# QZ1-boy/CDFO

Measured on NVIDIA B200. Metric: HR frames/sec, 1080p x4 LD-QP37, higher is better.
Workload: dtype bf16

## Files before the change

cdfo_b200/config.py:

```python
import os

tensor_core = True

dcn_gather = "tex"

conv_pair = os.environ.get("CDFO_CONV_PAIR", "1") != "0"

conv_fold_half = os.environ.get("CDFO_CONV_FOLD_HALF", "1") != "0"

conv_parity_planes = os.environ.get("CDFO_CONV_PARITY_PLANES", "1") != "0"
trunk_fused_resample = os.environ.get("CDFO_TRUNK_FUSED_RESAMPLE", "1") != "0"

head_dual = os.environ.get("CDFO_HEAD_DUAL", "1") != "0"

fused_head_dcn = os.environ.get("CDFO_FUSED_HEAD_DCN", "1") != "0"

features_c8 = os.environ.get("CDFO_FEATURES_C8", "1") != "0"
mdta_c8 = os.environ.get("CDFO_MDTA_C8", "1") != "0"
trunk_compose_1x1 = os.environ.get("CDFO_TRUNK_COMPOSE_1X1", "1") != "0"
trunk_fused_upsample = os.environ.get("CDFO_TRUNK_FUSED_UPSAMPLE", "1") != "0"
lra_logits_from_prior = os.environ.get("CDFO_LRA_LOGITS_FROM_PRIOR", "1") != "0"
```

cdfo_b200/csrc/lra.cu:

```cuda
#include <cuda.h>
#include <cstring>

#include "cdfo_common.cuh"
#include "sm100_ptx.cuh"

namespace cdfo {

__device__ __forceinline__ float warp_max(float v) {
#pragma unroll
  for (int o = 16; o > 0; o >>= 1) v = fmaxf(v, __shfl_xor_sync(0xffffffffu, v, o));
  return v;
}
__device__ __forceinline__ float warp_sum(float v) {
#pragma unroll
  for (int o = 16; o > 0; o >>= 1) v += __shfl_xor_sync(0xffffffffu, v, o);
  return v;
}

__global__ void lra_mask_kernel(const float *__restrict__ u, const float *__restrict__ vmax, const float *__restrict__ qv,
                                uint8_t *__restrict__ midx, float *__restrict__ qsel, int HW) {
  __shared__ float vm[64];
  const int b = blockIdx.y;
  if (threadIdx.x < 64) vm[threadIdx.x] = vmax[b * 64 + threadIdx.x];
  __syncthreads();
// ... 641 lines not shown
    for (int r = 0; r < 2; ++r) {
      l_run[r] += __shfl_xor_sync(0xffffffffu, l_run[r], 1);
      l_run[r] += __shfl_xor_sync(0xffffffffu, l_run[r], 2);
    }
    const float inv0 = 1.f / l_run[0], inv1 = 1.f / l_run[1];
    const int h0 = q0 + g, h1 = q0 + g + 8;
#pragma unroll
    for (int n = 0; n < 8; ++n) {
      if (h0 < H) *reinterpret_cast<float2 *>(long_out + (((size_t)b * H + h0) * W + w) * 64 + 8 * n + 2 * tq) = make_float2(o[n][0] * inv0, o[n][1] * inv0);
      if (h1 < H) *reinterpret_cast<float2 *>(long_out + (((size_t)b * H + h1) * W + w) * 64 + 8 * n + 2 * tq) = make_float2(o[n][2] * inv1, o[n][3] * inv1);
    }
  }
}

constexpr int kWinThreads = 256;
__global__ void __launch_bounds__(kWinThreads) lra_win_kernel(const float *__restrict__ qv, const uint8_t *__restrict__ midx,
                                                             float *__restrict__ loc_out, int H, int W) {
  extern __shared__ __align__(16) float sm[];
  float *q = sm;
  float *v = q + 64 * kLd;
  float *Ps = v + 64 * kLd;
  const int b = blockIdx.z, wy = blockIdx.y, wx = blockIdx.x;
  const int HW = H * W;
  const int tid = threadIdx.x;
  static_assert(kWinThreads == 256, "one token and 16 + 16 channels per thread");
  {
    const int tok = tid & 63, cg = tid >> 6;
    const int h = wy * 8 + (tok >> 3), w = wx * 8 + (tok & 7);
    const size_t pix = (size_t)h * W + w;
    const int cm = midx[(size_t)b * HW + pix];
    const float *qp = qv + ((size_t)b * 128 + cg) * HW + pix;
    float qr[16], vv[16];
#pragma unroll
    for (int k = 0; k < 16; ++k) {
      qr[k] = __ldg(qp + (size_t)(4 * k) * HW);
      vv[k] = __ldg(qp + (size_t)(64 + 4 * k) * HW);
    }
#pragma unroll
    for (int k = 0; k < 16; ++k) {
      const int c = 4 * k + cg;
      q[tok * kLd + c] = cm == c ? 0.f : qr[k];
      v[tok * kLd + c] = vv[k];
    }
  }
  __syncthreads();
  const float *Kcur = q;
  flash_block_fp32_kptr(q, &Kcur, v, Ps, 64, [&](int) {}, [&](int tok, int c4, float4 val) {
    const int h = wy * 8 + (tok >> 3), w = wx * 8 + (tok & 7);
    *reinterpret_cast<float4 *>(loc_out + (((size_t)b * H + h) * W + w) * 64 + c4) = val;
  });
}

constexpr int kWinTcThreads = 128, kWinLd = 36;
__global__ void __launch_bounds__(kWinTcThreads, 6) lra_win_tc_kernel(const float *__restrict__ qv, const uint8_t *__restrict__ midx,
                                                                      float *__restrict__ loc_out, int H, int W) {
  __shared__ uint32_t Qh[64 * kWinLd], Ql[64 * kWinLd], Vt[64 * kWinLd], Vl[64 * kWinLd];
  const int b = blockIdx.z, wy = blockIdx.y, wx = blockIdx.x;
  const int HW = H * W;
  const int tid = threadIdx.x, lane = tid & 31, warp = tid >> 5, g = lane >> 2, tq = lane & 3;
  {
    const int tok = tid & 63, half = tid >> 6;
    const int h = wy * 8 + (tok >> 3), w = wx * 8 + (tok & 7);
    const size_t pix = (size_t)h * W + w;
    const int cm = midx[(size_t)b * HW + pix];
    const float *qp = qv + ((size_t)b * 128 + half * 32) * HW + pix;
#pragma unroll 4
    for (int k = 0; k < 16; ++k) {
      const int c = half * 32 + 2 * k;
      float q0 = __ldg(qp + (size_t)(2 * k) * HW), q1 = __ldg(qp + (size_t)(2 * k + 1) * HW);
      if (cm == c) q0 = 0.f;
      if (cm == c + 1) q1 = 0.f;
      const __nv_bfloat16 h0 = __float2bfloat16_rn(q0), h1 = __float2bfloat16_rn(q1);
      Qh[tok * kWinLd + (c >> 1)] = pack_bf16x2(__bfloat162float(h0), __bfloat162float(h1));
      Ql[tok * kWinLd + (c >> 1)] = pack_bf16x2(q0 - __bfloat162float(h0), q1 - __bfloat162float(h1));
      const float v0 = __ldg(qp + (size_t)(64 + 2 * k) * HW), v1 = __ldg(qp + (size_t)(64 + 2 * k + 1) * HW);
      const __nv_bfloat16 vh0 = __float2bfloat16_rn(v0), vh1 = __float2bfloat16_rn(v1);
      reinterpret_cast<__nv_bfloat16 *>(Vt)[(c * kWinLd) * 2 + tok] = vh0;
      reinterpret_cast<__nv_bfloat16 *>(Vt)[((c + 1) * kWinLd) * 2 + tok] = vh1;
      reinterpret_cast<__nv_bfloat16 *>(Vl)[(c * kWinLd) * 2 + tok] = __float2bfloat16_rn(v0 - __bfloat162float(vh0));
      reinterpret_cast<__nv_bfloat16 *>(Vl)[((c + 1) * kWinLd) * 2 + tok] = __float2bfloat16_rn(v1 - __bfloat162float(vh1));
    }
  }
  __syncthreads();
  const int q0r = warp * 16;
  uint32_t ah[4][4], al[4][4];
#pragma unroll
  for (int s = 0; s < 4; ++s) {
    ah[s][0] = Qh[(q0r + g) * kWinLd + 8 * s + tq];      ah[s][1] = Qh[(q0r + g + 8) * kWinLd + 8 * s + tq];
    ah[s][2] = Qh[(q0r + g) * kWinLd + 8 * s + tq + 4];  ah[s][3] = Qh[(q0r + g + 8) * kWinLd + 8 * s + tq + 4];
    al[s][0] = Ql[(q0r + g) * kWinLd + 8 * s + tq];      al[s][1] = Ql[(q0r + g + 8) * kWinLd + 8 * s + tq];
    al[s][2] = Ql[(q0r + g) * kWinLd + 8 * s + tq + 4];  al[s][3] = Ql[(q0r + g + 8) * kWinLd + 8 * s + tq + 4];
  }
  float sc[8][4];
#pragma unroll
  for (int n = 0; n < 8; ++n) {
#pragma unroll
    for (int i = 0; i < 4; ++i) sc[n][i] = 0.f;
    const uint32_t *kh_ = Qh + (8 * n + g) * kWinLd + tq, *kl_ = Ql + (8 * n + g) * kWinLd + tq;
#pragma unroll
    for (int s = 0; s < 4; ++s) {
      const uint32_t bh0 = kh_[8 * s], bh1 = kh_[8 * s + 4];
      mma_bf16(sc[n], al[s], bh0, bh1);
      mma_bf16(sc[n], ah[s], kl_[8 * s], kl_[8 * s + 4]);
      mma_bf16(sc[n], ah[s], bh0, bh1);
    }
  }
  float mx[2] = {-INFINITY, -INFINITY}, sum[2] = {0.f, 0.f};
#pragma unroll
  for (int n = 0; n < 8; ++n) {
    mx[0] = fmaxf(mx[0], fmaxf(sc[n][0], sc[n][1]));
    mx[1] = fmaxf(mx[1], fmaxf(sc[n][2], sc[n][3]));
  }
#pragma unroll
  for (int r = 0; r < 2; ++r) {
    mx[r] = fmaxf(mx[r], __shfl_xor_sync(0xffffffffu, mx[r], 1));
    mx[r] = fmaxf(mx[r], __shfl_xor_sync(0xffffffffu, mx[r], 2));
  }
#pragma unroll
  for (int n = 0; n < 8; ++n) {
    sc[n][0] = expf(sc[n][0] - mx[0]); sc[n][1] = expf(sc[n][1] - mx[0]);
    sc[n][2] = expf(sc[n][2] - mx[1]); sc[n][3] = expf(sc[n][3] - mx[1]);
    sum[0] += sc[n][0] + sc[n][1];
    sum[1] += sc[n][2] + sc[n][3];
  }
  float o[8][4];
#pragma unroll
  for (int n = 0; n < 8; ++n)
#pragma unroll
    for (int i = 0; i < 4; ++i) o[n][i] = 0.f;
#pragma unroll
  for (int s = 0; s < 4; ++s) {
    uint32_t ap[4], apl[4];
#pragma unroll
    for (int i = 0; i < 4; ++i) {
      const float p0 = sc[2 * s + (i >> 1)][2 * (i & 1)], p1 = sc[2 * s + (i >> 1)][2 * (i & 1) + 1];
      const float h0 = __bfloat162float(__float2bfloat16_rn(p0)), h1 = __bfloat162float(__float2bfloat16_rn(p1));
      ap[i] = pack_bf16x2(h0, h1);
      apl[i] = pack_bf16x2(p0 - h0, p1 - h1);
    }
    const uint32_t *vr = Vt + g * kWinLd + 8 * s + tq, *vl = Vl + g * kWinLd + 8 * s + tq;
#pragma unroll
    for (int n = 0; n < 8; ++n) {
      const uint32_t b0 = vr[8 * n * kWinLd], b1 = vr[8 * n * kWinLd + 4];
      mma_bf16(o[n], apl, b0, b1);
      mma_bf16(o[n], ap, vl[8 * n * kWinLd], vl[8 * n * kWinLd + 4]);
      mma_bf16(o[n], ap, b0, b1);
    }
  }
#pragma unroll
  for (int r = 0; r < 2; ++r) {
    sum[r] += __shfl_xor_sync(0xffffffffu, sum[r], 1);
    sum[r] += __shfl_xor_sync(0xffffffffu, sum[r], 2);
  }
  const float inv0 = 1.f / sum[0], inv1 = 1.f / sum[1];
  const int t0 = q0r + g, t1 = t0 + 8;
  float *d0 = loc_out + (((size_t)b * H + wy * 8 + (t0 >> 3)) * W + wx * 8 + (t0 & 7)) * 64 + 2 * tq;
  float *d1 = loc_out + (((size_t)b * H + wy * 8 + (t1 >> 3)) * W + wx * 8 + (t1 & 7)) * 64 + 2 * tq;
#pragma unroll
  for (int n = 0; n < 8; ++n) {
    *reinterpret_cast<float2 *>(d0 + 8 * n) = make_float2(o[n][0] * inv0, o[n][1] * inv0);
    *reinterpret_cast<float2 *>(d1 + 8 * n) = make_float2(o[n][2] * inv1, o[n][3] * inv1);
  }
}

}

using namespace cdfo;

typedef CUresult (*LraEncodeTiledFn)(CUtensorMap *, CUtensorMapDataType, cuuint32_t, void *, const cuuint64_t *, const cuuint64_t *,
                                     const cuuint32_t *, const cuuint32_t *, CUtensorMapInterleave, CUtensorMapSwizzle,
                                     CUtensorMapL2promotion, CUtensorMapFloatOOBfill);
static LraEncodeTiledFn lra_encode_tiled_fn() {
  static LraEncodeTiledFn fn = nullptr;
  if (!fn) {
    void *ptr = nullptr;
    cudaDriverEntryPointQueryResult q;
    if (cudaGetDriverEntryPoint("cuTensorMapEncodeTiled", &ptr, cudaEnableDefault, &q) == cudaSuccess && q == cudaDriverEntryPointSuccess)
      fn = reinterpret_cast<LraEncodeTiledFn>(ptr);
  }
  return fn;
}

static bool g_lra_row_tma = true;
extern "C" int cdfo_lra_set_row_tma(int on) {
  g_lra_row_tma = on != 0;
  return CDFO_OK;
}
static bool g_lra_col_tf32 = false;
static bool g_lra_col_tc = true;
static bool g_lra_win_tc = true;
extern "C" int cdfo_lra_set_col_precision(int tf32) {
  g_lra_col_tf32 = tf32 != 0;
  return CDFO_OK;
}
extern "C" int cdfo_lra_set_col_tcgen05(int on) {
  g_lra_col_tc = on != 0;
  return CDFO_OK;
}
extern "C" int cdfo_lra_set_win_tensor_core(int on) {
  g_lra_win_tc = on != 0;
  return CDFO_OK;
}

extern "C" size_t cdfo_lra_workspace_bytes(int B, int H, int W) {
  const size_t P = (size_t)B * H * W;
  return P * (1 + 4) + 3 * P * 64 * 4 + 256;
}

static int lra_run(const float *qv, const float *u, const float *vmax, const float *x, const float *x2, const float *tables,
                   float beta, float bh, const float *fuse_w, const float *fuse_b, float *out, void *out_c8, int out_channels,
                   int channel0, void *workspace, int B, int H, int W, void *stream);

extern "C" int cdfo_lra_fwd(const float *qv, const float *u, const float *vmax, const float *x, const float *x2, const float *tables,
                            float beta, float bh, const float *fuse_w, const float *fuse_b, float *out, void *workspace, int B,
                            int H, int W, void *stream) {
  return lra_run(qv, u, vmax, x, x2, tables, beta, bh, fuse_w, fuse_b, out, nullptr, 0, 0, workspace, B, H, W, stream);
}

extern "C" int cdfo_lra_c8_fwd(const float *qv, const float *u, const float *vmax, const float *x, const float *x2, const float *tables,
                               float beta, float bh, const float *fuse_w, const float *fuse_b, void *out_c8, int out_channels,
                               int channel0, void *workspace, int B, int H, int W, void *stream) {
  CDFO_REQUIRE(out_c8 && ((uintptr_t)out_c8 & 15) == 0, CDFO_ERR_NULL, "cdfo_lra_c8_fwd: out_c8 must be a 16-byte aligned pointer");
  CDFO_REQUIRE(out_channels % 8 == 0 && channel0 % 8 == 0 && channel0 >= 0 && channel0 + 64 <= out_channels, CDFO_ERR_SHAPE,
               "cdfo_lra_c8_fwd: channels [%d, %d) do not fit %d output channels (multiples of 8)", channel0, channel0 + 64, out_channels);
  return lra_run(qv, u, vmax, x, x2, tables, beta, bh, fuse_w, fuse_b, nullptr, out_c8, out_channels, channel0, workspace, B, H, W, stream);
}

static int lra_run(const float *qv, const float *u, const float *vmax, const float *x, const float *x2, const float *tables,
                   float beta, float bh, const float *fuse_w, const float *fuse_b, float *out, void *out_c8, int out_channels,
                   int channel0, void *workspace, int B, int H, int W, void *stream) {
  CDFO_REQUIRE(qv && u && vmax && x && tables && fuse_w && fuse_b && (out || out_c8) && workspace, CDFO_ERR_NULL, "cdfo_lra_fwd: NULL pointer");
  CDFO_REQUIRE(B > 0 && B <= 65535 && H > 0 && W > 0 && H % 8 == 0 && W % 8 == 0, CDFO_ERR_SHAPE,
               "cdfo_lra_fwd: H and W must be multiples of the window size 8 (got %d x %d)", H, W);
  cudaStream_t s = (cudaStream_t)stream;
  const size_t P = (size_t)B * H * W;
  const int HW = H * W;
  uint8_t *ws = (uint8_t *)workspace;
  float *qsel = (float *)ws;
  float *vrow_t = qsel + P;
  float *long_out = vrow_t + P * 64;
  float *loc_out = long_out + P * 64;
  uint8_t *midx = (uint8_t *)(loc_out + P * 64);
  LraTables t{tables, tables + 9, tables + 18, tables + 82, beta, bh};

  lra_mask_kernel<<<dim3(ceil_div(HW, 128), B), 128, 0, s>>>(u, vmax, qv, midx, qsel, HW);

  const int Wk = (W + 63) & ~63;
  const size_t row_smem = ((size_t)Wk * kLd + 4096 + 3 * (size_t)Wk + 64 + kRowThreads + 2 * (size_t)Wk) * 4;
  const int Hk = (H + 63) & ~63;
  const size_t col_v = (size_t)Hk * kLd > (size_t)(H + 8) * 64 ? (size_t)Hk * kLd : (size_t)(H + 8) * 64;
  const size_t col_smem = ((size_t)Hk * kLd + col_v) * 4;
  const size_t win_smem = (size_t)3 * 64 * kLd * 4;
  const int kDynMax = 224 * 1024;
  CDFO_REQUIRE(row_smem <= (size_t)kDynMax && col_smem <= (size_t)kDynMax, CDFO_ERR_UNSUPPORTED,
               "cdfo_lra_fwd: frame %d x %d exceeds the shared-memory row/column buffers (W <= 704, H <= 384)", H, W);
  static bool attr = false;
  if (!attr) {
    cudaError_t e1 = cudaFuncSetAttribute(lra_row_kernel<false>, cudaFuncAttributeMaxDynamicSharedMemorySize, kDynMax);
    if (e1 == cudaSuccess) e1 = cudaFuncSetAttribute(lra_row_kernel<true>, cudaFuncAttributeMaxDynamicSharedMemorySize, kDynMax);
    cudaError_t e2 = cudaFuncSetAttribute(lra_col_kernel, cudaFuncAttributeMaxDynamicSharedMemorySize, kDynMax);
    if (e2 == cudaSuccess) e2 = cudaFuncSetAttribute(lra_col_bf16_kernel, cudaFuncAttributeMaxDynamicSharedMemorySize, kDynMax);
    cudaError_t e3 = cudaFuncSetAttribute(lra_win_kernel, cudaFuncAttributeMaxDynamicSharedMemorySize, (int)win_smem);
    if (e1 != cudaSuccess || e2 != cudaSuccess || e3 != cudaSuccess)
      return fail(CDFO_ERR_CUDA, "cdfo_lra_fwd: cudaFuncSetAttribute failed: %s", cudaGetErrorString(e1 != cudaSuccess ? e1 : (e2 != cudaSuccess ? e2 : e3)));
    attr = true;
  }
  {
    CUtensorMap qm;
    memset(&qm, 0, sizeof(qm));
    bool row_tma = g_lra_row_tma && W % 4 == 0 && ((uintptr_t)qv & 15) == 0 && row_smem + kRowRawBytes <= (size_t)kDynMax;
    if (row_tma) {
      static LraEncodeTiledFn enc = lra_encode_tiled_fn();
      if (enc) {
        const cuuint64_t gdim[3] = {(cuuint64_t)W, (cuuint64_t)H, (cuuint64_t)B * 128};
        const cuuint64_t gstr[2] = {(cuuint64_t)W * 4, (cuuint64_t)H * W * 4};
        const cuuint32_t box[3] = {kRowPiece, 1, 64};
        const cuuint32_t estr[3] = {1, 1, 1};
        CUresult cr = enc(&qm, CU_TENSOR_MAP_DATA_TYPE_FLOAT32, 3, const_cast<float *>(qv), gdim, gstr, box, estr, CU_TENSOR_MAP_INTERLEAVE_NONE,
                          CU_TENSOR_MAP_SWIZZLE_NONE, CU_TENSOR_MAP_L2_PROMOTION_L2_128B, CU_TENSOR_MAP_FLOAT_OOB_FILL_NONE);
        CDFO_REQUIRE(cr == CUDA_SUCCESS, CDFO_ERR_CUDA, "cuTensorMapEncodeTiled(qv rows) failed with CUresult %d", (int)cr);
      } else {
        row_tma = false;
      }
    }
    if (row_tma) lra_row_kernel<true><<<dim3(H, B), kRowThreads, row_smem + kRowRawBytes, s>>>(qm, qv, midx, qsel, vrow_t, t, H, W);
    else lra_row_kernel<false><<<dim3(H, B), kRowThreads, row_smem, s>>>(qm, qv, midx, qsel, vrow_t, t, H, W);
  }
  int col_done = 0;
  if (!g_lra_col_tf32 && g_lra_col_tc) {
    col_done = lra_col_sm100_launch(vrow_t, midx, qsel, long_out, t, B, H, W, s);
    if (col_done < 0) return col_done;
  }
  if (col_done) {
  } else if (g_lra_col_tf32) {
    lra_col_kernel<<<dim3(W, B), kColThreads, col_smem, s>>>(vrow_t, midx, qsel, long_out, t, H, W);
  } else {
    const size_t col16_smem = ((size_t)Hk * kQw + 64 * ((size_t)Hk / 2 + 4) + 2 * (size_t)(H + 8) + 16) * 4;
    lra_col_bf16_kernel<<<dim3(W, B), kColThreads, col16_smem, s>>>(vrow_t, midx, qsel, long_out, t, H, W);
  }
  if (g_lra_win_tc) lra_win_tc_kernel<<<dim3(W / 8, H / 8, B), kWinTcThreads, 0, s>>>(qv, midx, loc_out, H, W);
  else lra_win_kernel<<<dim3(W / 8, H / 8, B), kWinThreads, win_smem, s>>>(qv, midx, loc_out, H, W);
  if (int rc = check_launch("cdfo_lra_fwd")) return rc;
  return pointwise_conv(long_out, loc_out, fuse_w, fuse_b, x, x2, out, B, 128, 64, HW, 0, 1, s, out_c8, out_channels, channel0);
}
```

cdfo_b200/hotpath.py:

```python
import ctypes

import torch
import torch.nn.functional as F

from . import _lib, config, conv, dcn_sm100


def _lrelu(x):
    return F.leaky_relu(x, 0.1)


def _c(mod, x, **kw):
    return F.conv2d(x, mod.weight, mod.bias, **kw)


def _pkey(*params):
    return tuple((p.data_ptr(), str(p.device), p._version, p.dtype) for p in params)


def _module_cache(mod, slot, key, build):
    store = mod.__dict__.setdefault("_cdfo_derived", {})
    hit = store.get(slot)
    if hit is not None and hit[0] == key:
        return hit[1]
# ... 157 lines not shown
        k1 = tapm.sum(dim=1)
        r = tapm @ tapm.t()
        tab = torch.cat([kw, kh, k1, r.reshape(-1)]).float().contiguous()
        return tab, float(mod.directW1_conv.bias.detach()), float(mod.directH1_conv.bias.detach())
    return _module_cache(mod, "lra_tables", _pkey(mod.directW1_conv.weight, mod.directH1_conv.weight, mod.directW1_conv.bias,
                                                   mod.directH1_conv.bias), build)


@torch.no_grad()
def mask_logits(mod, v):
    B, C, H, W = v.shape
    if C != 64:
        raise _lib.CdfoError("mask_logits: 64 channels expected")
    c2, c3 = mod.conv_du_re._modules["2"], mod.conv_du_re2._modules["0"]
    ws = torch.empty(_lib.lib().cdfo_lra_mask_logits_workspace_bytes(B, H, W), dtype=torch.uint8, device=v.device)
    vmax = torch.empty((B, 64), dtype=torch.float32, device=v.device)
    _lib.call("cdfo_lra_mask_logits_fwd", _lib.ptr(_f32(v)), _lib.ptr(_f32(c2.weight)), _lib.ptr(_f32(c2.bias)), _lib.ptr(_f32(c3.weight).reshape(64, 64)),
              _lib.ptr(_f32(c3.bias)), _lib.ptr(vmax), _lib.ptr(ws), B, H, W, _lib.stream_ptr(v.device))
    return vmax


def _pointwise(in1, in2, weight, bias, act, mode=0, resid1=None, resid2=None):
    B, K, H, W = in1.shape
    Co = weight.size(0)
    out = torch.empty((B, Co, H, W), dtype=torch.float32, device=in1.device)
    _lib.call("cdfo_pointwise_conv_fwd", _lib.ptr(in1), _lib.ptr(in2), _lib.ptr(_f32(weight).reshape(Co, -1)), _lib.ptr(None if bias is None else _f32(bias)),
              _lib.ptr(resid1), _lib.ptr(resid2), _lib.ptr(out), B, K, Co, H, W, int(act), int(mode), _lib.stream_ptr(in1.device))
    return out


@torch.no_grad()
def long_range_attention(mod, res, x, u, x2=None, out8=None, channel0=0, res_prior=None):
    B, C, H, W = x.shape
    x = _f32(x)
    x2 = None if x2 is None else _f32(x2)
    du0 = mod.conv_du_re._modules["0"]
    if res_prior is not None:
        pc, rms1 = res_prior

        def build():
            w1 = du0.weight.detach().float().reshape(64, 64)
            return (w1 @ pc.weight.detach().float().reshape(64, 9)).contiguous(), (w1 @ pc.bias.detach().float() + du0.bias.detach().float()).contiguous()
        wv, bv = _module_cache(mod, "du0_after_prior", _pkey(du0.weight, du0.bias, pc.weight, pc.bias), build)
        rms1 = _f32(rms1)
        v = torch.empty((B, 64, H, W), dtype=torch.float32, device=x.device)
        _lib.call("cdfo_prior_conv_act_fwd", _lib.ptr(rms1), _lib.ptr(wv), _lib.ptr(bv), _lib.ptr(v), B, 64, H, W, 1, _lib.stream_ptr(x.device))
    else:
        v = _pointwise(_f32(res), None, du0.weight, du0.bias, act=1)
    vmax = mask_logits(mod, v)
    qv = _pointwise(x, x2, mod.input_conv.weight, mod.input_conv.bias, act=0)
    nbytes = _lib.lib().cdfo_lra_workspace_bytes(B, H, W)
    ws = torch.empty(nbytes, dtype=torch.uint8, device=x.device)
    tab, beta, bh = _lra_tap_tables(mod)
    if out8 is not None:
        if out8.dtype != torch.bfloat16 or not out8.is_contiguous() or out8.dim() != 5 or (out8.size(0), out8.size(2), out8.size(3), out8.size(4)) != (B, H, W, 8):
            raise _lib.CdfoError("long_range_attention: out8 must be a contiguous bf16 c8 tensor of the same batch and size")
        _lib.call("cdfo_lra_c8_fwd", _lib.ptr(qv), _lib.ptr(u.contiguous()), _lib.ptr(vmax), _lib.ptr(x), _lib.ptr(x2), _lib.ptr(tab),
                  ctypes.c_float(beta), ctypes.c_float(bh),
                  _lib.ptr(_f32(mod.fuse.weight).reshape(64, 128)), _lib.ptr(_f32(mod.fuse.bias)),
                  _lib.ptr(out8), out8.size(1) * 8, int(channel0), _lib.ptr(ws), B, H, W, _lib.stream_ptr(x.device))
        return out8
    out = torch.empty_like(x)
    _lib.call("cdfo_lra_fwd", _lib.ptr(qv), _lib.ptr(u.contiguous()), _lib.ptr(vmax), _lib.ptr(x), _lib.ptr(x2), _lib.ptr(tab),
              ctypes.c_float(beta), ctypes.c_float(bh),
              _lib.ptr(_f32(mod.fuse.weight).reshape(64, 128)), _lib.ptr(_f32(mod.fuse.bias)),
              _lib.ptr(out), _lib.ptr(ws), B, H, W, _lib.stream_ptr(x.device))
    return out


@torch.no_grad()
def prior_conv(conv_mod, x):
    B, C, H, W = x.shape
    if C != 1:
        raise _lib.CdfoError("prior_conv: one-channel input expected")
    x = _f32(x)
    Co = conv_mod.weight.size(0)
    y = torch.empty((B, Co, H, W), dtype=torch.float32, device=x.device)
    _lib.call("cdfo_prior_conv_fwd", _lib.ptr(x), _lib.ptr(_f32(conv_mod.weight)), _lib.ptr(_f32(conv_mod.bias)), _lib.ptr(y), B, Co, H, W,
              _lib.stream_ptr(x.device))
    return y


_SLOT = (0, 1, 2, 4, 5, 6)


@torch.no_grad()
def align_and_fuse(model, center, fea_nb, ufs_nb, rms_nb, mv_nb, u_nb, B):
    H, W = center.shape[2:]
    c8_align = (config.mdta_c8 and model.alignment == "mv_dcn" and config.dcn_gather == "tex" and config.fused_head_dcn
                and model.MV_deform_align.deformable_groups == 16)
    if c8_align:
        from . import features
        ufs_prior = features.prior_conv_c8(model.conv_expand_ufs, ufs_nb, lrelu=False)
    else:
        ufs_prior = prior_conv(model.conv_expand_ufs, ufs_nb)
    rms_prior = prior_conv(model.conv_expand_rms, rms_nb)
    runs = fea_nb if isinstance(fea_nb, (tuple, list)) else (fea_nb,)
    cat8 = torch.empty((6 * B, 16, H, W, 8), dtype=torch.bfloat16, device=center.device)
    off = 0
    for run in runs:
        sl = slice(off, off + run.size(0))
        long_range_attention(model.RDAB, rms_prior[sl], run, u_nb[sl], x2=rms_prior[sl], out8=cat8[sl], channel0=64,
                             res_prior=(model.conv_expand_rms, rms_nb[sl]) if config.lra_logits_from_prior else None)
        conv.to_c8(run, out=cat8[sl], channel0=0)
        off += run.size(0)
    fr = model.conv_expand_fea_r
# ... 139 lines not shown
```

include/cdfo_b200.h:

```cpp
#ifndef CDFO_B200_H_
#define CDFO_B200_H_

#include <stddef.h>
#include <stdint.h>

#ifdef __cplusplus
extern "C" {
#endif

typedef enum cdfo_status {
  CDFO_OK = 0,
  CDFO_ERR_SHAPE = -1,
  CDFO_ERR_NULL = -2,
  CDFO_ERR_CUDA = -3,
  CDFO_ERR_UNSUPPORTED = -4,
  CDFO_ERR_NO_DEVICE = -5
} cdfo_status;

typedef enum cdfo_dtype { CDFO_F32 = 0, CDFO_F16 = 1, CDFO_BF16 = 2 } cdfo_dtype;
#define CDFO_FIELDS_F16X4 16

const char *cdfo_last_error(void);
int cdfo_version(void);
int cdfo_device_ok(int dev);
// ... 32 lines not shown
                           long long fields_bstride, void *stream);
int cdfo_dcn_tex_sm100_set_fields_path(int use_tma);
int cdfo_dcn_tex_sm100_stacked_fwd(const void *x_q4t, const void *fields, const float *mv, const void *wpk, const float *bias,
                                   void *y_stack, int n_seq, int n_groups, int stack_chunks, const int *group_chunk, int H,
                                   int W, int dg, int x_batch, void *stream);
int cdfo_dcn_tex_sm100_pack_weight(const float *w, void *wpk, void *stream);
int cdfo_mv_head_dcn_fused_sm100_fwd(const void *z_c8, const void *head_wpk, const float *head_bias, float magnitude,
                                     const void *x_q4t, const float *mv, const void *dcn_wpk, const float *dcn_bias, void *y,
                                     void *fields_out, int B, int H, int W, int out_mode, int x_batch, int num_ctas, void *stream);
int cdfo_mv_head_dcn_fused_sm100_stacked_fwd(const void *z_c8, const void *head_wpk, const float *head_bias, float magnitude,
                                             const void *x_q4t, const float *mv, const void *dcn_wpk, const float *dcn_bias,
                                             void *y_stack, int n_seq, int n_groups, int stack_chunks, const int *group_chunk,
                                             int H, int W, int x_batch, void *stream);
int cdfo_pack_q4t(const float *x_nchw, void *x_q4t, int B, int C, int H, int W, void *stream);
int cdfo_q4t_pitch(int W);
size_t cdfo_q4t_bytes(int B, int C, int H, int W);
int cdfo_conv3x3_sm100_fwd(const void *x_c8, const void *wpk, const float *bias, const void *resid_c8, void *y,
                           int B, int Cin, int Cout, int H, int W, int act, int out_mode, void *stream);
int cdfo_mv_offset_head_sm100_fwd(const void *z_c8, const void *wpk, const float *bias, const void *first, void *out,
                                  int B, int Cin, int dg, int H, int W, float magnitude, void *stream);
int cdfo_mv_offset_head_dual_sm100_fwd(const void *z_c8, const void *wpk, const float *bias, void *out, int B, int Cin, int dg, int H,
                                       int W, float magnitude, void *stream);
int cdfo_conv_last_skip_sm100_fwd(const void *x_c8, const void *wpk, const float *bias, const float *lr, float *y, int B,
                                  int Cin, int H, int W, void *stream);
int cdfo_conv3x3_sm100_pack_weight(const float *w, void *wpk, int Cout, int Cin, void *stream);
int cdfo_conv_sm100_fwd(const void *x_c8, const void *wpk, const float *bias, const void *resid_c8, void *y, int B, int Cin,
                        int Cout, int H, int W, int ksize, int act, int out_mode, void *stream);
int cdfo_conv_sm100_pack_weight(const float *w, void *wpk, int Cout, int Cin, int ksize, void *stream);
size_t cdfo_conv_sm100_weight_bytes(int Cout, int Cin, int ksize);
size_t cdfo_conv3x3_sm100_weight_bytes(int Cout, int Cin);
int cdfo_conv3x3_sm100_ntile(int Cout, int Cin);
int cdfo_mdta_fwd(const float *x, int x_batch, const float *extra, const float *pred, const float *flow,
                  const float *fusion_w, const float *du_w1, const float *du_b1, const float *du_w2, const float *du_b2,
                  const float *temperature, const float *proj_w, int heads, int mode, void *out, float *ca_sums,
                  void *workspace, int B, int H, int W, void *stream);
int cdfo_mdta_c8_fwd(const void *x_c8, int x_batch, const void *extra_c8, const void *pred_c8, const float *flow, const float *fusion_w,
                     const float *du_w1, const float *du_b1, const float *du_w2, const float *du_b2, const float *temperature,
                     const float *proj_w, int heads, void *out_c8, void *workspace, int B, int H, int W, void *stream);
size_t cdfo_mdta_workspace_bytes(int B, int H, int W, int heads);
int cdfo_mdta_parts(int B);
int cdfo_channel_gate_fwd(const float *partial_sums, int parts, const float *w1, const float *b1, const float *w2,
                          const float *b2, float *gate, int B, int C, int Cmid, int HW, void *stream);
int cdfo_pack_c8_scaled(const float *x_nchw, const float *scale, void *x_c8, int B, int C, int H, int W, void *stream);
int cdfo_unpack_c8_add(const void *x_c8, const float *add_nchw, int add_batch, float *y_nchw, int B, int C, int H, int W,
                       void *stream);
int cdfo_resample_c8(const void *a, const void *b, const void *base, void *y, int B, int C, int Ho, int Wo, int mode, void *stream);
int cdfo_lra_fwd(const float *qv, const float *u, const float *vmax, const float *x, const float *x2, const float *tables,
                 float beta, float bh, const float *fuse_w, const float *fuse_b, float *out, void *workspace, int B, int H, int W,
                 void *stream);
int cdfo_lra_set_col_precision(int tf32);
int cdfo_lra_set_col_tcgen05(int on);
int cdfo_lra_set_win_tensor_core(int on);
int cdfo_lra_set_row_tma(int on);
int cdfo_lra_c8_fwd(const float *qv, const float *u, const float *vmax, const float *x, const float *x2, const float *tables,
                    float beta, float bh, const float *fuse_w, const float *fuse_b, void *out_c8, int out_channels, int channel0,
                    void *workspace, int B, int H, int W, void *stream);
int cdfo_pointwise_conv_fwd(const float *in1, const float *in2, const float *w, const float *bias, const float *resid1,
                            const float *resid2, float *out, int B, int K, int Co, int H, int W, int act, int mode, void *stream);
int cdfo_pointwise_conv_c8_fwd(const float *in1, const float *in2, const float *w, const float *bias, const float *resid1,
                               const float *resid2, void *out_c8, int B, int K, int Co, int H, int W, int act, int mode,
                               int out_channels, int channel0, void *stream);
size_t cdfo_lra_workspace_bytes(int B, int H, int W);
int cdfo_layernorm_c_fwd(const void *x, const float *gamma, const float *beta, void *y, int B, int C, int H, int W, float eps,
                         int dtype, void *stream);
int cdfo_dwconv3x3_fwd(const void *x, const float *w, void *y, int B, int C, int H, int W, int dtype, void *stream);
int cdfo_mdta_gram_fwd(const void *qk, float *partial, int B, int Ctot, int H, int W, int parts, int dtype, void *stream);
int cdfo_conv3x3_pair_sm100_supported(int Cout, int Cin);
size_t cdfo_conv3x3_pair_sm100_weight_bytes(int Cout, int Cin);
int cdfo_conv3x3_pair_sm100_pack_weight(const float *w, void *wpk, int Cout, int Cin, void *stream);
int cdfo_conv3x3_pair_sm100_fwd(const void *x_c8, const void *wpk, const float *bias, const void *resid_c8, void *y_c8, int B, int Cin,
                                int Cout, int H, int W, int act, void *stream);
int cdfo_conv3x3_pair_sm100_planes_fwd(const void *x_c8, const void *wpk, const float *bias, const void *resid_c8, void *y, int B,
                                       int Cin, int Cout, int H, int W, int act, int y_planes, void *stream);
int cdfo_conv3x3_pair_sm100_edge_fwd(const void *x_c8, const void *wpk, const float *bias, const float *bias_edge, const void *resid_c8,
                                     void *y, int B, int Cin, int Cout, int H, int W, int act, int y_planes, void *stream);
int cdfo_conv3x3_pair_sm100_up2_fwd(const void *x8_1x, const void *wpk, const float *bias, const float *bias_edge, void *y, int B, int Cin,
                                    int Cout, int H2, int W2, int act, int y_planes, void *stream);
int cdfo_conv4x4s2_pair_sm100_supported(int Cout, int Cin);
size_t cdfo_conv4x4s2_pair_sm100_weight_bytes(int Cin);
int cdfo_conv4x4s2_pair_sm100_pack_weight(const float *w3, void *wpk, int Cin, void *stream);
int cdfo_conv4x4s2_pair_sm100_fwd(const void *x_c8, const void *wpk, const float *bias, const void *resid_c8, void *y_c8, int B, int Cin,
                                  int H_in, int W_in, void *stream);
int cdfo_conv4x4s2_pair_sm100_planes_fwd(const void *x, const void *wpk, const float *bias, const void *resid_c8, void *y_c8, int B,
                                         int Cin, int H_in, int W_in, int x_planes, void *stream);
int cdfo_conv4x4s2_pair_sm100_block_fwd(const void *x, const void *wpk, const float *bias, const void *resid_c8, const void *up_c8,
                                        void *y_c8, void *half_c8, int B, int Cin, int H_in, int W_in, int x_planes, void *stream);
int cdfo_planes_to_unit_f32(const void *src, int src_kind, float *dst, int n_planes, int H_in, int W, int H_out, void *stream);
int cdfo_sr_to_u8(const float *sr, uint8_t *out, int n_planes, int H_in, int W, int H_out, void *stream);
size_t cdfo_psnr_ssim_workspace_bytes(int B, int H, int W, int border);
int cdfo_psnr_ssim_u8(const uint8_t *res, const uint8_t *gt, int B, int H, int W, int border, double *frame_out, double *accum,
                      void *workspace, void *stream);
int cdfo_umma_selftest(const void *A, const void *B, float *D, int swap_lbo_sbo, void *stream);

size_t cdfo_lra_mask_logits_workspace_bytes(int B, int H, int W);
int cdfo_lra_mask_logits_fwd(const float *v, const float *w2, const float *b2, const float *w3, const float *b3, float *vmax,
                             void *workspace, int B, int H, int W, void *stream);
int cdfo_lra_set_logit_tma(int on);

int cdfo_prior_conv_c8_fwd(const float *x, const float *w, const float *bias, void *y_c8, int B, int Co, int H, int W, int lrelu, void *stream);
int cdfo_layernorm_c8_fwd(const void *x_c8, const float *gamma, const float *beta, void *y_c8, int B, int H, int W, float eps, void *stream);
int cdfo_dwconv3x3_c8_fwd(const void *x_c8, const float *w, void *y_c8, int B, int C, int H, int W, void *stream);
int cdfo_mdta_gram_c8_fwd(const void *qkv_c8, float *partial, int B, int C, int H, int W, int parts, void *stream);
int cdfo_mdta_fold_fwd(const float *partial, const float *temperature, const float *project_out, float *M, int B, int parts, void *stream);
int cdfo_mdta_apply_c8_fwd(const void *qkv_c8, int C, int v_channel0, const float *M, const void *x1_c8, const void *x2_c8, void *out1_c8,
                           void *out2_c8, int B, int H, int W, void *stream);
int cdfo_conv16_c8_fwd(const void *x_c8, const float *w, const float *bias, void *y_c8, int B, int Hi, int Wi, int Ho, int Wo, int y_channels,
// ... 8 lines not shown
```

Measured before the change: 89.24.

## Stream LRA window attention through persistent TMA double-buffered kernel

Adds a persistent window-attention kernel that loads each 8x8x128 qv window with TMA into a double-buffered shared staging area, prefetching the next window while the current one is converted and attended. It replaces the strided per-channel __ldg gathers and the one-block-per-window launch with a grid of two blocks per SM. The trade is 64KB of dynamic shared memory per block, which lowers occupancy to 2 blocks/SM, plus extra block-wide syncs per window. The old kernel remains as a fallback when the flag is off or alignment or tensor-map encoding is unavailable.

```diff
diff --git a/cdfo_b200/config.py b/cdfo_b200/config.py
--- a/cdfo_b200/config.py
+++ b/cdfo_b200/config.py
@@ -20,3 +20,4 @@
 trunk_compose_1x1 = os.environ.get("CDFO_TRUNK_COMPOSE_1X1", "1") != "0"
 trunk_fused_upsample = os.environ.get("CDFO_TRUNK_FUSED_UPSAMPLE", "1") != "0"
 lra_logits_from_prior = os.environ.get("CDFO_LRA_LOGITS_FROM_PRIOR", "1") != "0"
+lra_streamed = os.environ.get("CDFO_LRA_STREAMED", "1") != "0"
diff --git a/cdfo_b200/csrc/lra.cu b/cdfo_b200/csrc/lra.cu
--- a/cdfo_b200/csrc/lra.cu
+++ b/cdfo_b200/csrc/lra.cu
@@ -717,12 +717,113 @@
 }
 
 constexpr int kWinTcThreads = 128, kWinLd = 36;
+
+__device__ __forceinline__ void win_tc_fill_q(uint32_t *Qh, uint32_t *Ql, int tok, int c, int cm, float q0, float q1) {
+  if (cm == c) q0 = 0.f;
+  if (cm == c + 1) q1 = 0.f;
+  const __nv_bfloat16 h0 = __float2bfloat16_rn(q0), h1 = __float2bfloat16_rn(q1);
+  Qh[tok * kWinLd + (c >> 1)] = pack_bf16x2(__bfloat162float(h0), __bfloat162float(h1));
+  Ql[tok * kWinLd + (c >> 1)] = pack_bf16x2(q0 - __bfloat162float(h0), q1 - __bfloat162float(h1));
+}
+__device__ __forceinline__ void win_tc_fill_v(uint32_t *Vt, uint32_t *Vl, int tok, int c, float v0, float v1) {
+  const __nv_bfloat16 vh0 = __float2bfloat16_rn(v0), vh1 = __float2bfloat16_rn(v1);
+  reinterpret_cast<__nv_bfloat16 *>(Vt)[(c * kWinLd) * 2 + tok] = vh0;
+  reinterpret_cast<__nv_bfloat16 *>(Vt)[((c + 1) * kWinLd) * 2 + tok] = vh1;
+  reinterpret_cast<__nv_bfloat16 *>(Vl)[(c * kWinLd) * 2 + tok] = __float2bfloat16_rn(v0 - __bfloat162float(vh0));
+  reinterpret_cast<__nv_bfloat16 *>(Vl)[((c + 1) * kWinLd) * 2 + tok] = __float2bfloat16_rn(v1 - __bfloat162float(vh1));
+}
+
+__device__ __forceinline__ void win_tc_attend(const uint32_t *Qh, const uint32_t *Ql, const uint32_t *Vt, const uint32_t *Vl,
+                                              float *__restrict__ loc_out, int b, int wy, int wx, int H, int W) {
+  const int tid = threadIdx.x, lane = tid & 31, warp = tid >> 5, g = lane >> 2, tq = lane & 3;
+  const int q0r = warp * 16;
+  uint32_t ah[4][4], al[4][4];
+#pragma unroll
+  for (int s = 0; s < 4; ++s) {
+    ah[s][0] = Qh[(q0r + g) * kWinLd + 8 * s + tq];      ah[s][1] = Qh[(q0r + g + 8) * kWinLd + 8 * s + tq];
+    ah[s][2] = Qh[(q0r + g) * kWinLd + 8 * s + tq + 4];  ah[s][3] = Qh[(q0r + g + 8) * kWinLd + 8 * s + tq + 4];
+    al[s][0] = Ql[(q0r + g) * kWinLd + 8 * s + tq];      al[s][1] = Ql[(q0r + g + 8) * kWinLd + 8 * s + tq];
+    al[s][2] = Ql[(q0r + g) * kWinLd + 8 * s + tq + 4];  al[s][3] = Ql[(q0r + g + 8) * kWinLd + 8 * s + tq + 4];
+  }
+  float sc[8][4];
+#pragma unroll
+  for (int n = 0; n < 8; ++n) {
+#pragma unroll
+    for (int i = 0; i < 4; ++i) sc[n][i] = 0.f;
+    const uint32_t *kh_ = Qh + (8 * n + g) * kWinLd + tq, *kl_ = Ql + (8 * n + g) * kWinLd + tq;
+#pragma unroll
+    for (int s = 0; s < 4; ++s) {
+      const uint32_t bh0 = kh_[8 * s], bh1 = kh_[8 * s + 4];
+      mma_bf16(sc[n], al[s], bh0, bh1);
+      mma_bf16(sc[n], ah[s], kl_[8 * s], kl_[8 * s + 4]);
+      mma_bf16(sc[n], ah[s], bh0, bh1);
+    }
+  }
+  float mx[2] = {-INFINITY, -INFINITY}, sum[2] = {0.f, 0.f};
+#pragma unroll
+  for (int n = 0; n < 8; ++n) {
+    mx[0] = fmaxf(mx[0], fmaxf(sc[n][0], sc[n][1]));
+    mx[1] = fmaxf(mx[1], fmaxf(sc[n][2], sc[n][3]));
+  }
+#pragma unroll
+  for (int r = 0; r < 2; ++r) {
+    mx[r] = fmaxf(mx[r], __shfl_xor_sync(0xffffffffu, mx[r], 1));
+    mx[r] = fmaxf(mx[r], __shfl_xor_sync(0xffffffffu, mx[r], 2));
+  }
+#pragma unroll
+  for (int n = 0; n < 8; ++n) {
+    sc[n][0] = expf(sc[n][0] - mx[0]); sc[n][1] = expf(sc[n][1] - mx[0]);
+    sc[n][2] = expf(sc[n][2] - mx[1]); sc[n][3] = expf(sc[n][3] - mx[1]);
+    sum[0] += sc[n][0] + sc[n][1];
+    sum[1] += sc[n][2] + sc[n][3];
+  }
+  float o[8][4];
+#pragma unroll
+  for (int n = 0; n < 8; ++n)
+#pragma unroll
+    for (int i = 0; i < 4; ++i) o[n][i] = 0.f;
+#pragma unroll
+  for (int s = 0; s < 4; ++s) {
+    uint32_t ap[4], apl[4];
+#pragma unroll
+    for (int i = 0; i < 4; ++i) {
+      const float p0 = sc[2 * s + (i >> 1)][2 * (i & 1)], p1 = sc[2 * s + (i >> 1)][2 * (i & 1) + 1];
+      const float h0 = __bfloat162float(__float2bfloat16_rn(p0)), h1 = __bfloat162float(__float2bfloat16_rn(p1));
+      ap[i] = pack_bf16x2(h0, h1);
+      apl[i] = pack_bf16x2(p0 - h0, p1 - h1);
+    }
+    const uint32_t *vr = Vt + g * kWinLd + 8 * s + tq, *vl = Vl + g * kWinLd + 8 * s + tq;
+#pragma unroll
+    for (int n = 0; n < 8; ++n) {
+      const uint32_t b0 = vr[8 * n * kWinLd], b1 = vr[8 * n * kWinLd + 4];
+      mma_bf16(o[n], apl, b0, b1);
+      mma_bf16(o[n], ap, vl[8 * n * kWinLd], vl[8 * n * kWinLd + 4]);
+      mma_bf16(o[n], ap, b0, b1);
+    }
+  }
+#pragma unroll
+  for (int r = 0; r < 2; ++r) {
+    sum[r] += __shfl_xor_sync(0xffffffffu, sum[r], 1);
+    sum[r] += __shfl_xor_sync(0xffffffffu, sum[r], 2);
+  }
+  const float inv0 = 1.f / sum[0], inv1 = 1.f / sum[1];
+  const int t0 = q0r + g, t1 = t0 + 8;
+  float *d0 = loc_out + (((size_t)b * H + wy * 8 + (t0 >> 3)) * W + wx * 8 + (t0 & 7)) * 64 + 2 * tq;
+  float *d1 = loc_out + (((size_t)b * H + wy * 8 + (t1 >> 3)) * W + wx * 8 + (t1 & 7)) * 64 + 2 * tq;
+#pragma unroll
+  for (int n = 0; n < 8; ++n) {
+    *reinterpret_cast<float2 *>(d0 + 8 * n) = make_float2(o[n][0] * inv0, o[n][1] * inv0);
+    *reinterpret_cast<float2 *>(d1 + 8 * n) = make_float2(o[n][2] * inv1, o[n][3] * inv1);
+  }
+}
+
+
 __global__ void __launch_bounds__(kWinTcThreads, 6) lra_win_tc_kernel(const float *__restrict__ qv, const uint8_t *__restrict__ midx,
                                                                       float *__restrict__ loc_out, int H, int W) {
   __shared__ uint32_t Qh[64 * kWinLd], Ql[64 * kWinLd], Vt[64 * kWinLd], Vl[64 * kWinLd];
   const int b = blockIdx.z, wy = blockIdx.y, wx = blockIdx.x;
   const int HW = H * W;
-  const int tid = threadIdx.x, lane = tid & 31, warp = tid >> 5, g = lane >> 2, tq = lane & 3;
+  const int tid = threadIdx.x;
   {
     const int tok = tid & 63, half = tid >> 6;
     const int h = wy * 8 + (tok >> 3), w = wx * 8 + (tok & 7);
@@ -731,100 +832,52 @@
     const float *qp = qv + ((size_t)b * 128 + half * 32) * HW + pix;
 #pragma unroll 4
     for (int k = 0; k < 16; ++k) {
-      const int c = half * 32 + 2 * k;
-      float q0 = __ldg(qp + (size_t)(2 * k) * HW), q1 = __ldg(qp + (size_t)(2 * k + 1) * HW);
-      if (cm == c) q0 = 0.f;
-      if (cm == c + 1) q1 = 0.f;
-      const __nv_bfloat16 h0 = __float2bfloat16_rn(q0), h1 = __float2bfloat16_rn(q1);
-      Qh[tok * kWinLd + (c >> 1)] = pack_bf16x2(__bfloat162float(h0), __bfloat162float(h1));
-      Ql[tok * kWinLd + (c >> 1)] = pack_bf16x2(q0 - __bfloat162float(h0), q1 - __bfloat162float(h1));
-      const float v0 = __ldg(qp + (size_t)(64 + 2 * k) * HW), v1 = __ldg(qp + (size_t)(64 + 2 * k + 1) * HW);
-      const __nv_bfloat16 vh0 = __float2bfloat16_rn(v0), vh1 = __float2bfloat16_rn(v1);
-      reinterpret_cast<__nv_bfloat16 *>(Vt)[(c * kWinLd) * 2 + tok] = vh0;
-      reinterpret_cast<__nv_bfloat16 *>(Vt)[((c + 1) * kWinLd) * 2 + tok] = vh1;
-      reinterpret_cast<__nv_bfloat16 *>(Vl)[(c * kWinLd) * 2 + tok] = __float2bfloat16_rn(v0 - __bfloat162float(vh0));
-      reinterpret_cast<__nv_bfloat16 *>(Vl)[((c + 1) * kWinLd) * 2 + tok] = __float2bfloat16_rn(v1 - __bfloat162float(vh1));
-    }
-  }
-  __syncthreads();
-  const int q0r = warp * 16;
-  uint32_t ah[4][4], al[4][4];
-#pragma unroll
-  for (int s = 0; s < 4; ++s) {
-    ah[s][0] = Qh[(q0r + g) * kWinLd + 8 * s + tq];      ah[s][1] = Qh[(q0r + g + 8) * kWinLd + 8 * s + tq];
-    ah[s][2] = Qh[(q0r + g) * kWinLd + 8 * s + tq + 4];  ah[s][3] = Qh[(q0r + g + 8) * kWinLd + 8 * s + tq + 4];
-    al[s][0] = Ql[(q0r + g) * kWinLd + 8 * s + tq];      al[s][1] = Ql[(q0r + g + 8) * kWinLd + 8 * s + tq];
-    al[s][2] = Ql[(q0r + g) * kWinLd + 8 * s + tq + 4];  al[s][3] = Ql[(q0r + g + 8) * kWinLd + 8 * s + tq + 4];
-  }
-  float sc[8][4];
-#pragma unroll
-  for (int n = 0; n < 8; ++n) {
-#pragma unroll
-    for (int i = 0; i < 4; ++i) sc[n][i] = 0.f;
-    const uint32_t *kh_ = Qh + (8 * n + g) * kWinLd + tq, *kl_ = Ql + (8 * n + g) * kWinLd + tq;
-#pragma unroll
-    for (int s = 0; s < 4; ++s) {
-      const uint32_t bh0 = kh_[8 * s], bh1 = kh_[8 * s + 4];
-      mma_bf16(sc[n], al[s], bh0, bh1);
-      mma_bf16(sc[n], ah[s], kl_[8 * s], kl_[8 * s + 4]);
-      mma_bf16(sc[n], ah[s], bh0, bh1);
-    }
-  }
-  float mx[2] = {-INFINITY, -INFINITY}, sum[2] = {0.f, 0.f};
-#pragma unroll
-  for (int n = 0; n < 8; ++n) {
-    mx[0] = fmaxf(mx[0], fmaxf(sc[n][0], sc[n][1]));
-    mx[1] = fmaxf(mx[1], fmaxf(sc[n][2], sc[n][3]));
-  }
-#pragma unroll
-  for (int r = 0; r < 2; ++r) {
-    mx[r] = fmaxf(mx[r], __shfl_xor_sync(0xffffffffu, mx[r], 1));
-    mx[r] = fmaxf(mx[r], __shfl_xor_sync(0xffffffffu, mx[r], 2));
-  }
-#pragma unroll
-  for (int n = 0; n < 8; ++n) {
-    sc[n][0] = expf(sc[n][0] - mx[0]); sc[n][1] = expf(sc[n][1] - mx[0]);
-    sc[n][2] = expf(sc[n][2] - mx[1]); sc[n][3] = expf(sc[n][3] - mx[1]);
-    sum[0] += sc[n][0] + sc[n][1];
-    sum[1] += sc[n][2] + sc[n][3];
-  }
-  float o[8][4];
-#pragma unroll
-  for (int n = 0; n < 8; ++n)
-#pragma unroll
-    for (int i = 0; i < 4; ++i) o[n][i] = 0.f;
-#pragma unroll
-  for (int s = 0; s < 4; ++s) {
-    uint32_t ap[4], apl[4];
-#pragma unroll
-    for (int i = 0; i < 4; ++i) {
-      const float p0 = sc[2 * s + (i >> 1)][2 * (i & 1)], p1 = sc[2 * s + (i >> 1)][2 * (i & 1) + 1];
-      const float h0 = __bfloat162float(__float2bfloat16_rn(p0)), h1 = __bfloat162float(__float2bfloat16_rn(p1));
-      ap[i] = pack_bf16x2(h0, h1);
-      apl[i] = pack_bf16x2(p0 - h0, p1 - h1);
-    }
-    const uint32_t *vr = Vt + g * kWinLd + 8 * s + tq, *vl = Vl + g * kWinLd + 8 * s + tq;
-#pragma unroll
-    for (int n = 0; n < 8; ++n) {
-      const uint32_t b0 = vr[8 * n * kWinLd], b1 = vr[8 * n * kWinLd + 4];
-      mma_bf16(o[n], apl, b0, b1);
-      mma_bf16(o[n], ap, vl[8 * n * kWinLd], vl[8 * n * kWinLd + 4]);
-      mma_bf16(o[n], ap, b0, b1);
-    }
-  }
-#pragma unroll
-  for (int r = 0; r < 2; ++r) {
-    sum[r] += __shfl_xor_sync(0xffffffffu, sum[r], 1);
-    sum[r] += __shfl_xor_sync(0xffffffffu, sum[r], 2);
-  }
-  const float inv0 = 1.f / sum[0], inv1 = 1.f / sum[1];
-  const int t0 = q0r + g, t1 = t0 + 8;
-  float *d0 = loc_out + (((size_t)b * H + wy * 8 + (t0 >> 3)) * W + wx * 8 + (t0 & 7)) * 64 + 2 * tq;
-  float *d1 = loc_out + (((size_t)b * H + wy * 8 + (t1 >> 3)) * W + wx * 8 + (t1 & 7)) * 64 + 2 * tq;
-#pragma unroll
-  for (int n = 0; n < 8; ++n) {
-    *reinterpret_cast<float2 *>(d0 + 8 * n) = make_float2(o[n][0] * inv0, o[n][1] * inv0);
-    *reinterpret_cast<float2 *>(d1 + 8 * n) = make_float2(o[n][2] * inv1, o[n][3] * inv1);
+      win_tc_fill_q(Qh, Ql, tok, half * 32 + 2 * k, cm, __ldg(qp + (size_t)(2 * k) * HW), __ldg(qp + (size_t)(2 * k + 1) * HW));
+      win_tc_fill_v(Vt, Vl, tok, half * 32 + 2 * k, __ldg(qp + (size_t)(64 + 2 * k) * HW), __ldg(qp + (size_t)(64 + 2 * k + 1) * HW));
+    }
+  }
+  __syncthreads();
+  win_tc_attend(Qh, Ql, Vt, Vl, loc_out, b, wy, wx, H, W);
+}
+
+constexpr int kWinBoxFloats = 128 * 64;
+constexpr int kWinStreamSmem = 2 * kWinBoxFloats * 4 + 16;
+__global__ void __launch_bounds__(kWinTcThreads, 2) lra_win_tc_stream_kernel(const __grid_constant__ CUtensorMap qvmap,
+                                                                             const uint8_t *__restrict__ midx, float *__restrict__ loc_out,
+                                                                             int B, int H, int W) {
+  extern __shared__ __align__(128) float raw[];
+  __shared__ uint32_t Qh[64 * kWinLd], Ql[64 * kWinLd], Vt[64 * kWinLd], Vl[64 * kWinLd];
+  const uint32_t bar0 = ptx::smem_u32(raw + 2 * kWinBoxFloats);
+  const int nwx = W / 8, nwin_img = (H / 8) * nwx, n_win = B * nwin_img;
+  const int tid = threadIdx.x, tok = tid & 63, half = tid >> 6;
+  if (tid == 0) {
+    ptx::mbar_init(bar0, 1);
+    ptx::mbar_init(bar0 + 8, 1);
+    ptx::fence_mbar_init();
+  }
+  __syncthreads();
+  auto issue = [&](int win, int st) {
+    const int b = win / nwin_img, r = win - b * nwin_img, wy = r / nwx, wx = r - wy * nwx;
+    ptx::mbar_arrive_expect_tx(bar0 + 8 * st, kWinBoxFloats * 4);
+    ptx::tma_load_3d(ptx::smem_u32(raw + st * kWinBoxFloats), &qvmap, bar0 + 8 * st, wx * 8, wy * 8, b * 128);
+  };
+  if (tid == 0 && blockIdx.x < n_win) issue(blockIdx.x, 0);
+  int it = 0;
+  for (int win = blockIdx.x; win < n_win; win += gridDim.x, ++it) {
+    const int st = it & 1;
+    if (tid == 0 && win + (int)gridDim.x < n_win) issue(win + gridDim.x, st ^ 1);
+    const int b = win / nwin_img, r = win - b * nwin_img, wy = r / nwx, wx = r - wy * nwx;
+    const int cm = midx[((size_t)b * H + wy * 8 + (tok >> 3)) * W + wx * 8 + (tok & 7)];
+    ptx::mbar_wait_parked(bar0 + 8 * st, (it >> 1) & 1);
+    const float *rq = raw + st * kWinBoxFloats + half * 32 * 64 + tok;
+#pragma unroll 4
+    for (int k = 0; k < 16; ++k) {
+      win_tc_fill_q(Qh, Ql, tok, half * 32 + 2 * k, cm, rq[(2 * k) * 64], rq[(2 * k + 1) * 64]);
+      win_tc_fill_v(Vt, Vl, tok, half * 32 + 2 * k, rq[(64 + 2 * k) * 64], rq[(64 + 2 * k + 1) * 64]);
+    }
+    __syncthreads();
+    win_tc_attend(Qh, Ql, Vt, Vl, loc_out, b, wy, wx, H, W);
+    __syncthreads();
   }
 }
 
@@ -849,6 +902,11 @@
 static bool g_lra_row_tma = true;
 extern "C" int cdfo_lra_set_row_tma(int on) {
   g_lra_row_tma = on != 0;
+  return CDFO_OK;
+}
+static bool g_lra_streamed = true;
+extern "C" int cdfo_lra_set_streamed(int on) {
+  g_lra_streamed = on != 0;
   return CDFO_OK;
 }
 static bool g_lra_col_tf32 = false;
@@ -926,6 +984,7 @@
     cudaError_t e2 = cudaFuncSetAttribute(lra_col_kernel, cudaFuncAttributeMaxDynamicSharedMemorySize, kDynMax);
     if (e2 == cudaSuccess) e2 = cudaFuncSetAttribute(lra_col_bf16_kernel, cudaFuncAttributeMaxDynamicSharedMemorySize, kDynMax);
     cudaError_t e3 = cudaFuncSetAttribute(lra_win_kernel, cudaFuncAttributeMaxDynamicSharedMemorySize, (int)win_smem);
+    if (e3 == cudaSuccess) e3 = cudaFuncSetAttribute(lra_win_tc_stream_kernel, cudaFuncAttributeMaxDynamicSharedMemorySize, kWinStreamSmem);
     if (e1 != cudaSuccess || e2 != cudaSuccess || e3 != cudaSuccess)
       return fail(CDFO_ERR_CUDA, "cdfo_lra_fwd: cudaFuncSetAttribute failed: %s", cudaGetErrorString(e1 != cudaSuccess ? e1 : (e2 != cudaSuccess ? e2 : e3)));
     attr = true;
@@ -963,7 +1022,25 @@
     const size_t col16_smem = ((size_t)Hk * kQw + 64 * ((size_t)Hk / 2 + 4) + 2 * (size_t)(H + 8) + 16) * 4;
     lra_col_bf16_kernel<<<dim3(W, B), kColThreads, col16_smem, s>>>(vrow_t, midx, qsel, long_out, t, H, W);
   }
-  if (g_lra_win_tc) lra_win_tc_kernel<<<dim3(W / 8, H / 8, B), kWinTcThreads, 0, s>>>(qv, midx, loc_out, H, W);
+  static LraEncodeTiledFn win_enc = lra_encode_tiled_fn();
+  if (g_lra_streamed && g_lra_win_tc && win_enc && ((uintptr_t)qv & 15) == 0) {
+    int dev = 0, n_sm = 0;
+    cudaError_t e = cudaGetDevice(&dev);
+    if (e == cudaSuccess) e = cudaDeviceGetAttribute(&n_sm, cudaDevAttrMultiProcessorCount, dev);
+    if (e != cudaSuccess) return fail(CDFO_ERR_CUDA, "cdfo_lra_fwd: SM count query failed: %s", cudaGetErrorString(e));
+    CUtensorMap wm;
+    memset(&wm, 0, sizeof(wm));
+    const cuuint64_t gdim[3] = {(cuuint64_t)W, (cuuint64_t)H, (cuuint64_t)B * 128};
+    const cuuint64_t gstr[2] = {(cuuint64_t)W * 4, (cuuint64_t)H * W * 4};
+    const cuuint32_t box[3] = {8, 8, 128};
+    const cuuint32_t estr[3] = {1, 1, 1};
+    CUresult cr = win_enc(&wm, CU_TENSOR_MAP_DATA_TYPE_FLOAT32, 3, const_cast<float *>(qv), gdim, gstr, box, estr, CU_TENSOR_MAP_INTERLEAVE_NONE,
+                          CU_TENSOR_MAP_SWIZZLE_NONE, CU_TENSOR_MAP_L2_PROMOTION_L2_128B, CU_TENSOR_MAP_FLOAT_OOB_FILL_NONE);
+    CDFO_REQUIRE(cr == CUDA_SUCCESS, CDFO_ERR_CUDA, "cuTensorMapEncodeTiled(qv windows) failed with CUresult %d", (int)cr);
+    const int n_win = B * (H / 8) * (W / 8);
+    const int grid = n_win < 2 * n_sm ? n_win : 2 * n_sm;
+    lra_win_tc_stream_kernel<<<grid, kWinTcThreads, kWinStreamSmem, s>>>(wm, midx, loc_out, B, H, W);
+  } else if (g_lra_win_tc) lra_win_tc_kernel<<<dim3(W / 8, H / 8, B), kWinTcThreads, 0, s>>>(qv, midx, loc_out, H, W);
   else lra_win_kernel<<<dim3(W / 8, H / 8, B), kWinThreads, win_smem, s>>>(qv, midx, loc_out, H, W);
   if (int rc = check_launch("cdfo_lra_fwd")) return rc;
   return pointwise_conv(long_out, loc_out, fuse_w, fuse_b, x, x2, out, B, 128, 64, HW, 0, 1, s, out_c8, out_channels, channel0);
diff --git a/cdfo_b200/hotpath.py b/cdfo_b200/hotpath.py
--- a/cdfo_b200/hotpath.py
+++ b/cdfo_b200/hotpath.py
@@ -233,6 +233,7 @@
     nbytes = _lib.lib().cdfo_lra_workspace_bytes(B, H, W)
     ws = torch.empty(nbytes, dtype=torch.uint8, device=x.device)
     tab, beta, bh = _lra_tap_tables(mod)
+    _lib.call("cdfo_lra_set_streamed", int(config.lra_streamed))
     if out8 is not None:
         if out8.dtype != torch.bfloat16 or not out8.is_contiguous() or out8.dim() != 5 or (out8.size(0), out8.size(2), out8.size(3), out8.size(4)) != (B, H, W, 8):
             raise _lib.CdfoError("long_range_attention: out8 must be a contiguous bf16 c8 tensor of the same batch and size")
diff --git a/include/cdfo_b200.h b/include/cdfo_b200.h
--- a/include/cdfo_b200.h
+++ b/include/cdfo_b200.h
@@ -108,6 +108,7 @@
 int cdfo_lra_set_col_tcgen05(int on);
 int cdfo_lra_set_win_tensor_core(int on);
 int cdfo_lra_set_row_tma(int on);
+int cdfo_lra_set_streamed(int on);
 int cdfo_lra_c8_fwd(const float *qv, const float *u, const float *vmax, const float *x, const float *x2, const float *tables,
                     float beta, float bh, const float *fuse_w, const float *fuse_b, void *out_c8, int out_channels, int channel0,
                     void *workspace, int B, int H, int W, void *stream);
```

Result: no change. 89.50, median of 6 (+0.3%).
